# heliaxdev/kzg-setup-powersoftau

Hardware: AMD Instinct MI355X
Metric: G1+G2 points decompressed+checked/sec, 2^27 BLS12-381 PoT (higher is better)
Workload: dtype u32 (381-bit Montgomery, 14 x 28-bit limbs)

## Files before the change

### kzg-setup-powersoftau_amd/csrc/curve.hpp

```cpp
#pragma once
#include "fp381.hpp"

namespace kzgpot {

template <typename F>
struct jac {
  F x, y, z;
};

template <const auto& K>
KZG_DEV void f_subk(fp& r, const fp& a, const fp& b) { fp_subk_nr<K>(r, a, b); }
template <int S>
KZG_DEV void f_shl(fp& r, const fp& a) { fp_shl_nr<S>(r, a); }
KZG_DEV void f_mul_sub(fp& r, const fp& a, const fp& b, const fp& c, const fp& d) {
  fp nd;
  fp_negk_nr<BlsFp::KB_4_28>(nd, d);
  fp_mul_sum2(r, a, b, c, nd);
}

KZG_DEV void jac_dbl(jac<fp>& p) {
  fp a, b, d, e, t;
  fp_sqr(a, p.x);
  fp_sqr(b, p.y);
  fp_shl_nr<2>(t, p.x);
  fp_mul(d, t, b);
  fp_mul3_nr(e, a);
  fp_norm(e, e);
  fp_shl_nr<1>(t, p.y);
  fp_mul(p.z, t, p.z);
  fp_sqr(a, e);
  fp_shl_nr<1>(t, d);
  fp_subk_nr<BlsFp::KB_8_29>(p.x, a, t);
  fp_mul3_nr(t, d);
  fp_subk_nr<BlsFp::KB_8_30>(t, a, t);
  fp_mul_add8sqr(d, e, t, b);
  fp_negk_nr<BlsFp::KB_2_28>(p.y, d);
}

constexpr int F30_ZK = 16;
KZG_DEV void f_one(f30& r) { f30_set(r, ONE30); }

KZG_DEV void jac_dbl_w(jac<f30>& p) {
  f30 a, b, d, e, t;
  f30_sqr(a, p.x);
  f30_sqr(b, p.y);
  f30_mul(d, p.x, b);
  f30_mul3(e, a);
  f30_norm(e, e);
  f30_mul(p.z, p.y, p.z);
  f30_sqr<-2>(p.x, e, d);
  f30_sub(t, p.x, d);
  f30_norm<1>(t, t);
  f30_mul_addsqr(d, e, t, b);
  f30_neg(p.y, d);
}

KZG_DEV void jac_tpl_affine_w(jac<f30>& p) {
  f30 xx, yy, m, mm, s, e, ee, t, u, n;
  f30_sqr(xx, p.x);
  f30_sqr(yy, p.y);
  f30_sqr(t, yy);
  f30_mul3(m, xx);
  f30_norm(m, m);
  f30_sqr(mm, m);
  f30_mul(s, p.x, yy);
  f30_mul3(s, s);
  f30_norm(s, s);
  f30_sub(s, s, mm);
  f30_norm(e, s);
  f30_sqr(ee, e);
  f30_add(s, m, e);
  f30_norm(s, s);
  f30_sqr<-1, -1>(s, s, mm, ee);
  f30_sub(s, s, t);
  f30_norm(u, s);
  f30_neg(n, u);
  f30_mul_sum2(s, p.x, ee, yy, n);
  f30_norm<2>(p.x, s);
  f30_sub(t, t, u);
  f30_norm(t, t);
  f30_neg(n, ee);
  f30_mul_sum2(s, u, t, e, n);
  f30_mul(s, p.y, s);
  f30_norm<3>(p.y, s);
  f30_norm<1>(p.z, e);
}

template <typename Load>
KZG_DEV void jac_madd_w(jac<f30>& p, Load&& load) {
  f30 z1z1, h, r, t;
  {
    f30 x2, w2;
    load(x2, w2);
    f30_sqr(z1z1, p.z);
    f30_mul<-1>(h, x2, z1z1, p.x);
    f30_mul(t, w2, p.z);
    f30_mul<-1>(r, t, z1z1, p.y);
  }
  const bool z1zero = f30_is_zero<F30_ZK>(p.z);
  const bool same = !z1zero && f30_is_zero<F30_ZK>(h) && f30_is_zero<F30_ZK>(r);
  if (__builtin_expect(z1zero || same, 0)) {
    if (same) {
      jac_dbl_w(p);
    } else {
      load(p.x, p.y);
      f_one(p.z);
    }
    return;
  }
  f30 hh, j;
  f30_sqr(hh, h);
  f30_dbl(t, p.z);
  f30_mul(p.z, t, h);
  f30_norm<2>(hh, hh);
  f30_mul(j, h, hh);
  f30_mul(hh, p.x, hh);
  f30_sqr<-1, -2>(t, r, j, hh);
  f30_sub(hh, hh, t);
  f30_norm(hh, hh);
  f30_norm<1>(r, r);
  f30_norm<1>(h, p.y);
  f30_neg(j, j);
  f30_mul_sum2(p.y, r, hh, h, j);
  p.x = t;
}

template <const auto& K>
KZG_DEV void f2_mul_lz(fp2& r, const fp2& a, const fp2& b) {
  fp nb1, c0;
  fp_negk_nr<K>(nb1, b.c1);
  fp_mul_sum2(c0, a.c0, b.c0, a.c1, nb1);
  fp_mul_sum2(r.c1, a.c0, b.c1, a.c1, b.c0);
  r.c0 = c0;
}
template <const auto& K>
KZG_DEV void f2_sqr_lz(fp2& r, const fp2& a) {
  fp s, d, t;
  fp_add_nr(s, a.c0, a.c1);
  fp_subk_nr<K>(d, a.c0, a.c1);
  fp_shl_nr<1>(t, a.c0);
  fp_mul(r.c1, t, a.c1);
  fp_mul(r.c0, s, d);
}
template <const auto& K>
KZG_DEV void f2_subk(fp2& r, const fp2& a, const fp2& b) {
  fp_subk_nr<K>(r.c0, a.c0, b.c0);
  fp_subk_nr<K>(r.c1, a.c1, b.c1);
}
template <int S>
KZG_DEV void f2_shl(fp2& r, const fp2& a) {
  fp_shl_nr<S>(r.c0, a.c0);
  fp_shl_nr<S>(r.c1, a.c1);
}
KZG_DEV void f2_add_nr(fp2& r, const fp2& a, const fp2& b) {
  fp_add_nr(r.c0, a.c0, b.c0);
  fp_add_nr(r.c1, a.c1, b.c1);
}
KZG_DEV void f2_norm(fp2& r, const fp2& a) {
  fp_norm(r.c0, a.c0);
  fp_norm(r.c1, a.c1);
}

template <bool W = false>
KZG_DEV void jac_dbl(jac<fp2>& p) {
  fp2 b, a, d, t;
  if constexpr (W) {
    f2_sqr_lz<BlsFp::KB_32_29>(b, p.y);
    f2_mul_lz<BlsFp::KB_16_28>(p.z, p.y, p.z);
  } else {
    f2_sqr_lz<BlsFp::KB_32_28>(b, p.y);
    f2_shl<1>(t, p.y);
    f2_mul_lz<BlsFp::KB_16_28>(p.z, t, p.z);
  }
  f2_sqr_lz<BlsFp::KB_16_28>(a, p.x);
  if constexpr (W) {
    f2_mul_lz<BlsFp::KB_2_28>(d, p.x, b);
  } else {
    f2_shl<2>(t, p.x);
    f2_mul_lz<BlsFp::KB_2_28>(d, t, b);
  }
  fp_mul3_nr(a.c0, a.c0);
  fp_mul3_nr(a.c1, a.c1);
  f2_norm(a, a);
  f2_sqr_lz<BlsFp::KB_4_28>(t, a);
  f2_shl<1>(p.x, d);
  f2_subk<BlsFp::KB_4_29>(p.x, t, p.x);
  f2_norm(p.x, p.x);
  f2_subk<BlsFp::KB_8_28>(d, d, p.x);
  if constexpr (W) f2_shl<1>(a, a);
  fp u, s, n, c0;
  fp_negk_nr<BlsFp::KB_16_30>(u, d.c1);
  fp_add_nr(s, b.c0, b.c1);
  if constexpr (W) {
    fp_subk_nr<BlsFp::KB_2_28>(n, b.c1, b.c0);
    fp_norm(n, n);
  } else {
    fp_subk_nr<BlsFp::KB_2_28>(n, b.c0, b.c1);
    fp_norm(n, n);
    fp_shl_nr<3>(n, n);
    fp_negk_nr<BlsFp::KB_64_31>(n, n);
    fp_norm(n, n);
  }
  fp_mul_sum3(c0, a.c0, d.c0, a.c1, u, s, n);
  if constexpr (W) {
    fp_negk_nr<BlsFp::KB_2_28>(n, b.c1);
  } else {
    fp_shl_nr<3>(n, b.c1);
    fp_negk_nr<BlsFp::KB_16_31>(n, n);
    fp_norm(n, n);
  }
  fp_shl_nr<1>(s, b.c0);
  fp_mul_sum3(p.y.c1, a.c0, d.c1, a.c1, d.c0, s, n);
  p.y.c0 = c0;
}

template <bool W = false, typename Load>
KZG_DEV void jac_madd(jac<fp2>& p, Load&& load) {
  fp2 z1z1, h, r, t;
  {
    fp2 x2, y2;
    load(x2, y2);
    f2_sqr_lz<BlsFp::KB_16_28>(z1z1, p.z);
    f2_mul_lz<BlsFp::KB_2_28>(h, x2, z1z1);
    f2_subk<BlsFp::KB_32_28>(h, h, p.x);
    f2_norm(h, h);
    f2_mul_lz<BlsFp::KB_16_28>(t, y2, p.z);
    f2_mul_lz<BlsFp::KB_2_28>(t, t, z1z1);
    if constexpr (W)
      f2_subk<BlsFp::KB_32_29>(r, t, p.y);
    else
      f2_subk<BlsFp::KB_32_28>(r, t, p.y);
    f2_norm(r, r);
  }
  const bool z1zero = f_is_zero(p.z);
  const bool same = !z1zero && f_is_zero(h) && f_is_zero(r);
  if (__builtin_expect(z1zero || same, 0)) {
    if (same) {
      jac_dbl<W>(p);
    } else {
      load(p.x, p.y);
      f_one(p.z);
    }
    return;
  }
  fp2 hh, j;
  f2_sqr_lz<BlsFp::KB_64_28>(hh, h);
  f2_shl<1>(t, p.z);
  f2_mul_lz<BlsFp::KB_64_28>(p.z, t, h);
  f2_shl<2>(hh, hh);
  f2_mul_lz<BlsFp::KB_8_30>(j, h, hh);
  f2_mul_lz<BlsFp::KB_8_30>(hh, p.x, hh);
  f2_sqr_lz<BlsFp::KB_64_28>(t, r);
  if constexpr (!W) f2_shl<2>(t, t);
  f2_subk<BlsFp::KB_2_28>(t, t, j);
  f2_shl<1>(h, hh);
  f2_subk<BlsFp::KB_4_29>(t, t, h);
  f2_norm(t, t);
  f2_subk<BlsFp::KB_32_28>(hh, hh, t);
  f2_shl<1>(r, r);
  f2_mul_lz<BlsFp::KB_64_30>(hh, r, hh);
  f2_shl<1>(h, p.y);
  f2_mul_lz<BlsFp::KB_2_28>(j, h, j);
  f2_subk<BlsFp::KB_4_28>(p.y, hh, j);
  f2_norm(p.y, p.y);
  p.x = t;
}

template <typename Load>
KZG_DEV void jac_tpl_affine_w(jac<fp2>& p, Load&& load) {
  fp2 yy, m, s, ee, t;
  load(p.x, p.y);
  f2_sqr_lz<BlsFp::KB_2_28>(m, p.x);
  f2_sqr_lz<BlsFp::KB_4_29>(yy, p.y);
  f2_mul_lz<BlsFp::KB_2_28>(p.z, p.x, yy);
  fp_mul3_nr(m.c0, m.c0);
  fp_mul3_nr(m.c1, m.c1);
  f2_norm(m, m);
  f2_sqr_lz<BlsFp::KB_4_28>(t, m);
  fp_mul3_nr(p.z.c0, p.z.c0);
  fp_mul3_nr(p.z.c1, p.z.c1);
  f2_subk<BlsFp::KB_2_28>(p.z, p.z, t);
  f2_norm(p.z, p.z);
  f2_add_nr(s, m, p.z);
  f2_norm(s, s);
  f2_sqr_lz<BlsFp::KB_32_28>(s, s);
  f2_subk<BlsFp::KB_2_28>(s, s, t);
  f2_sqr_lz<BlsFp::KB_16_28>(ee, p.z);
  f2_subk<BlsFp::KB_4_28>(s, s, ee);
  f2_sqr_lz<BlsFp::KB_2_28>(t, yy);
  f2_subk<BlsFp::KB_2_28>(s, s, t);
  f2_norm(s, s);
  f2_subk<BlsFp::KB_64_28>(t, t, s);
  f2_norm(t, t);
  f2_mul_lz<BlsFp::KB_128_28>(t, s, t);
  f2_mul_lz<BlsFp::KB_64_28>(yy, yy, s);
  f2_mul_lz<BlsFp::KB_2_28>(m, p.z, ee);
  f2_subk<BlsFp::KB_2_28>(t, t, m);
  f2_norm(t, t);
  load(p.x, p.y);
  f2_mul_lz<BlsFp::KB_2_28>(p.x, p.x, ee);
  f2_subk<BlsFp::KB_2_28>(p.x, p.x, yy);
  f2_norm(p.x, p.x);
  f2_mul_lz<BlsFp::KB_8_28>(p.y, p.y, t);
}

template <typename F, typename Load>
KZG_DEV void jac_madd(jac<F>& p, Load&& load) {
  F z1z1, h, r, t;
  {
    F x2, y2;
    load(x2, y2);
    f_sqr(z1z1, p.z);
    f_mul(h, x2, z1z1);
    f_subk<BlsFp::KB_128_31>(h, h, p.x);
    f_norm(h, h);
    f_mul(t, y2, p.z);
    f_mul(t, t, z1z1);
    f_subk<BlsFp::KB_64_31>(r, t, p.y);
    f_norm(r, r);
  }
  const bool z1zero = f_is_zero(p.z);
  const bool same = !z1zero && f_is_zero(h) && f_is_zero(r);
  if (__builtin_expect(z1zero || same, 0)) {
    if (same) {
      jac_dbl(p);
    } else {
      load(p.x, p.y);
      f_one(p.z);
    }
    return;
  }
  F hh, j;
  f_sqr(hh, h);
  f_shl<1>(t, p.z);
  f_mul(p.z, t, h);
  f_shl<2>(hh, hh);
  f_norm(hh, hh);
  f_mul(j, h, hh);
  f_mul(hh, p.x, hh);
  f_sqr(t, r);
  f_shl<2>(t, t);
  f_subk<BlsFp::KB_32_28>(t, t, j);
  f_shl<1>(h, hh);
  f_subk<BlsFp::KB_64_29>(t, t, h);
  f_norm(t, t);
  f_subk<BlsFp::KB_128_28>(hh, hh, t);
  f_norm(hh, hh);
  f_shl<1>(r, r);
  f_shl<1>(h, p.y);
  f_mul_sub(p.y, r, hh, h, j);
  p.x = t;
}

template <typename F, typename Load>
KZG_DEV void mul_abs_u_affine(jac<F>& acc, Load&& load) {
  static_assert(((BLS_ABS_U >> (BLS_ABS_U_BITS - 2)) & 3) == 3, "|u| starts with the bits 11");
  if constexpr (__is_same(F, f30)) {
    load(acc.x, acc.y);
    jac_tpl_affine_w(acc);
#pragma unroll 1
    for (int b = BLS_ABS_U_BITS - 3; b >= 0; b--) {
      jac_dbl_w(acc);
      if ((BLS_ABS_U >> b) & 1) jac_madd_w(acc, load);
    }
  } else {
    static_assert(__is_same(F, fp2), "the fast ladders run on f30 (G1) and fp2 (G2)");
    auto loadw = [&](fp2& x, fp2& w) {
      load(x, w);
      f2_shl<1>(w, w);
    };
    jac_tpl_affine_w(acc, loadw);
#pragma unroll 1
    for (int b = BLS_ABS_U_BITS - 3; b >= 0; b--) {
      jac_dbl<true>(acc);
      if ((BLS_ABS_U >> b) & 1) jac_madd<true>(acc, loadw);
    }
  }
}
template <typename F>
KZG_DEV bool jac_eq_affine(const jac<F>& p, const F& x, const F& y) {
  F z2, t;
  f_sqr(z2, p.z);
  f_mul(t, x, z2);
  f_subk<BlsFp::KB_128_31>(t, t, p.x);
  bool ok = f_is_zero(t);
  f_mul(z2, z2, p.z);
  f_mul(t, y, z2);
  f_subk<BlsFp::KB_128_31>(t, t, p.y);
  ok = ok && f_is_zero(t);
  return ok && !f_is_zero(p.z);
}

KZG_DEV bool jac_eq_affine(const jac<fp2>& p, const fp2& x, const fp2& y) {
  fp2 z2, t;
  f2_sqr_lz<BlsFp::KB_16_28>(z2, p.z);
  f2_mul_lz<BlsFp::KB_2_28>(t, x, z2);
  f2_subk<BlsFp::KB_32_28>(t, t, p.x);
  bool ok = f_is_zero(t);
  f2_mul_lz<BlsFp::KB_16_28>(z2, z2, p.z);
  f2_mul_lz<BlsFp::KB_2_28>(t, y, z2);
  f2_subk<BlsFp::KB_32_29>(t, t, p.y);
  ok = ok && f_is_zero(t);
  return ok && !f_is_zero(p.z);
}

template <typename F, typename Load>
KZG_DEV bool in_subgroup_ref(Load&& load) {
  jac<F> acc;
  load(acc.x, acc.y);
  f_one(acc.z);
#pragma unroll 1
  for (int b = FR_R_BITS - 2; b >= 0; b--) {
    jac_dbl(acc);
    const uint32_t word = FR_R[b >> 5];
    if ((word >> (b & 31)) & 1) jac_madd(acc, load);
  }
  return f_is_zero(acc.z);
}

KZG_DEV bool jac_eq_affine(const jac<f30>& p, const f30& x, const f30& w) {
  f30 z2, t;
  f30_sqr(z2, p.z);
  f30_mul(t, x, z2);
  f30_sub(t, t, p.x);
  bool ok = f30_is_zero<F30_ZK>(t);
  f30_mul(z2, z2, p.z);
  f30_mul(t, w, z2);
  f30_sub(t, t, p.y);
  ok = ok && f30_is_zero<F30_ZK>(t);
  return ok && !f30_is_zero<F30_ZK>(p.z);
}

template <typename LoadRow, typename Park, typename LoadQZ>
KZG_DEV bool in_subgroup_fast_g1(LoadRow&& load_row, Park&& park, LoadQZ&& load_qz) {
  jac<f30> q;
  int src = 0;
  auto load = [&](f30& bx, f30& bw) { load_row(src, bx, bw); };
#pragma unroll 1
  for (int pass = 0; pass < 2; pass++) {
    src = __builtin_amdgcn_readfirstlane(pass);
    mul_abs_u_affine(q, load);
    if (pass == 0) park(q);
  }
  {
    f30 z;
    load_qz(z);
    f30_mul(q.z, q.z, z);
  }
  f30 x, w, beta;
  load_row(0, x, w);
  f30_set(beta, BETA30);
  f30_mul(x, x, beta);
  f30_neg(w, w);
  return jac_eq_affine(q, x, w);
}

KZG_DEV void g2_psi(fp2& x, fp2& y) {
  fp cx1, t;
  fp_set(cx1, FP_PSI_CX1);
  fp_mul(t, x.c1, cx1);
  fp_mul(x.c1, x.c0, cx1);
  x.c0 = t;
  fp2 cy;
  fp_set(cy.c0, FP_PSI_CY0);
  fp_set(cy.c1, FP_PSI_CY1);
  fp zero;
  fp_zero(zero);
  fp_sub_red(y.c1, zero, y.c1);
  f_mul(y, y, cy);
}

template <typename Load>
KZG_DEV bool in_subgroup_fast_g2(Load&& load) {
  jac<fp2> q;
  mul_abs_u_affine(q, load);
  fp2 x, y;
  load(x, y);
  g2_psi(x, y);
  fp2_neg_red(y, y);
  f2_shl<1>(y, y);
  return jac_eq_affine(q, x, y);
}

KZG_DEV void f_inv(fp& r, const fp& a) {
  fp t;
  fp_pow_pm3d4(t, a);
  fp_sqr(t, t);
  fp_sqr(t, t);
  fp_mul(r, t, a);
}
KZG_DEV void f_inv(fp2& r, const fp2& a) {
  fp n, t;
  fp_sqr(n, a.c0);
  fp_sqr(t, a.c1);
  fp_add(n, n, t);
  f_inv(n, n);
  fp_mul(r.c0, a.c0, n);
  fp_mul(t, a.c1, n);
  fp_zero(n);
  fp_sub_red(r.c1, n, t);
}

template <typename F>
KZG_DEV void to_affine(F& x, F& y, const jac<F>& p) {
  F zi, z2;
  f_inv(zi, p.z);
  f_sqr(z2, zi);
  f_mul(x, p.x, z2);
  f_mul(z2, z2, zi);
  f_mul(y, p.y, z2);
}

}
```

### kzg-setup-powersoftau_amd/csrc/fp381.hpp

```cpp
#pragma once
#include <hip/hip_runtime.h>
#include <stdint.h>

#include <utility>

#include "bls12_381_consts.hpp"
#include "bn254_consts.hpp"

#define KZG_DEV __device__ __forceinline__

#ifndef KZG_FPOP
#define KZG_FPOP(kind) ((void)0)
#endif

namespace kzgpot {

enum class FpOp { Mul, Sqr, MulSum2, MulSum3, MulAddSqr, Mul30, Sqr30, Mul30Sum2, Mul30AddSqr, Count };

constexpr uint32_t LMASK = (1u << 28) - 1;

template <class Tr>
struct Fe {
  uint32_t v[Tr::NL];
};
// ... 195 lines not shown
KZG_DEV void fp_mul3_nr(Fe<Tr>& r, const Fe<Tr>& a) {
#pragma unroll
  for (int i = 0; i < Tr::NL; i++) r.v[i] = (a.v[i] << 1) + a.v[i];
}
template <uint32_t C>
KZG_DEV uint32_t lit_sub(uint32_t b) {
  uint32_t r;
  asm("v_sub_u32_e32 %0, %1, %2" : "=v"(r) : "n"(C), "v"(b));
  return r;
}
template <uint32_t C>
KZG_DEV uint32_t lit_add(uint32_t a) {
  uint32_t r;
  asm("v_add_u32_e32 %0, %1, %2" : "=v"(r) : "n"(C), "v"(a));
  return r;
}
template <const auto& K, class Tr, size_t... I>
KZG_DEV void subk_lit(Fe<Tr>& r, const Fe<Tr>& a, const Fe<Tr>& b, std::index_sequence<I...>) {
  ((r.v[I] = lit_add<K[I]>(a.v[I]) - b.v[I]), ...);
}
template <const auto& K, class Tr, size_t... I>
KZG_DEV void negk_lit(Fe<Tr>& r, const Fe<Tr>& b, std::index_sequence<I...>) {
  ((r.v[I] = lit_sub<K[I]>(b.v[I])), ...);
}
template <const auto& K, class Tr>
KZG_DEV void fp_subk_nr(Fe<Tr>& r, const Fe<Tr>& a, const Fe<Tr>& b) {
  subk_lit<K>(r, a, b, std::make_index_sequence<Tr::NL>{});
}
template <const auto& K, class Tr>
KZG_DEV void fp_negk_nr(Fe<Tr>& r, const Fe<Tr>& b) {
  negk_lit<K>(r, b, std::make_index_sequence<Tr::NL>{});
}
template <class Tr>
KZG_DEV void fp_norm(Fe<Tr>& r, const Fe<Tr>& a) {
  uint32_t c = 0;
#pragma unroll
  for (int i = 0; i < Tr::NL - 1; i++) {
    const uint32_t t = a.v[i] + c;
    r.v[i] = t & Tr::MASK;
    c = t >> Tr::LB;
  }
  r.v[Tr::NL - 1] = a.v[Tr::NL - 1] + c;
}
template <class Tr>
KZG_DEV void fp_select(Fe<Tr>& r, bool c, const Fe<Tr>& a, const Fe<Tr>& b) {
#pragma unroll
  for (int i = 0; i < Tr::NL; i++) r.v[i] = c ? a.v[i] : b.v[i];
}

template <class Tr>
KZG_DEV void fp_half(Fe<Tr>& r, const Fe<Tr>& a) {
  const uint32_t odd = 0u - (a.v[0] & 1u);
  Fe<Tr> t;
  uint32_t c = 0;
#pragma unroll
  for (int i = 0; i < Tr::NL - 1; i++) {
    const uint32_t s = a.v[i] + (Tr::P[i] & odd) + c;
    t.v[i] = s & Tr::MASK;
    c = s >> Tr::LB;
  }
  t.v[Tr::NL - 1] = a.v[Tr::NL - 1] + (Tr::P[Tr::NL - 1] & odd) + c;
#pragma unroll
  for (int i = 0; i < Tr::NL - 1; i++) r.v[i] = (t.v[i] >> 1) | ((t.v[i + 1] & 1u) << (Tr::LB - 1));
  r.v[Tr::NL - 1] = t.v[Tr::NL - 1] >> 1;
}

template <class Tr>
KZG_DEV bool fp_sub_const_borrow(Fe<Tr>& d, const Fe<Tr>& a, const uint32_t (&k)[Tr::NL]) {
  int32_t br = 0;
#pragma unroll
  for (int i = 0; i < Tr::NL; i++) {
    const int32_t t = (int32_t)a.v[i] - (int32_t)k[i] + br;
    d.v[i] = (uint32_t)t & Tr::MASK;
    br = t >> Tr::LB;
  }
  return br != 0;
}
template <class Tr>
KZG_DEV void fp_reduce_once(Fe<Tr>& r, const Fe<Tr>& a) {
  Fe<Tr> d;
  const bool b = fp_sub_const_borrow(d, a, Tr::P);
  fp_select(r, b, a, d);
}
template <class Tr>
KZG_DEV void fp_reduce_canon(Fe<Tr>& r, const Fe<Tr>& a) {
  Fe<Tr> x = a, d;
#define KZG_RED_STEP(K)                          \
  {                                              \
    const bool b = fp_sub_const_borrow(d, x, K); \
    fp_select(x, b, x, d);                       \
  }
  KZG_RED_STEP(Tr::P_X128)
  KZG_RED_STEP(Tr::P_X64)
  KZG_RED_STEP(Tr::P_X32)
  KZG_RED_STEP(Tr::P_X16)
  KZG_RED_STEP(Tr::P_X8)
  KZG_RED_STEP(Tr::P_X4)
  KZG_RED_STEP(Tr::P_X2)
  KZG_RED_STEP(Tr::P_X1)
#undef KZG_RED_STEP
  r = x;
}
template <class Tr>
KZG_DEV void fp_canon(Fe<Tr>& r, const Fe<Tr>& a) {
  Fe<Tr> n;
  fp_norm(n, a);
  fp_reduce_canon(r, n);
}
template <class Tr>
KZG_DEV bool fp_is_zero_canon(const Fe<Tr>& c) {
  uint32_t o = 0;
#pragma unroll
  for (int i = 0; i < Tr::NL; i++) o |= c.v[i];
  return o == 0;
}
template <class Tr>
KZG_DEV bool fp_is_zero(const Fe<Tr>& a) {
  constexpr int N = Tr::NL;
  const uint32_t kc = ((a.v[0] & Tr::MASK) * (0u - Tr::PINV)) & Tr::MASK;
  const bool maybe = kc < 256u;
  if (__builtin_amdgcn_ballot_w64(maybe) == 0) return false;
  if (!maybe) return false;
  Fe<Tr> n;
  fp_norm(n, a);
  const uint32_t k = (uint32_t)((double)(n.v[N - 1] + 1u) * Tr::INV_RHO);
  uint64_t c = 0;
  uint32_t diff = 0;
#pragma unroll
  for (int i = 0; i < N - 1; i++) {
    c += (uint64_t)k * Tr::P[i];
    diff |= ((uint32_t)c & Tr::MASK) ^ n.v[i];
    c >>= Tr::LB;
  }
  c += (uint64_t)k * Tr::P[N - 1];
  diff |= (uint32_t)c ^ n.v[N - 1];
  return diff == 0;
}
template <class Tr>
KZG_DEV bool fp_eq(const Fe<Tr>& a, const Fe<Tr>& b) {
  Fe<Tr> d;
  fp_subk_nr<Tr::KB_EQ>(d, a, b);
  return fp_is_zero(d);
}
template <class Tr>
KZG_DEV bool fp_lt_canon(const Fe<Tr>& a, const Fe<Tr>& b) {
  Fe<Tr> d;
  return fp_sub_const_borrow(d, a, b.v);
}
template <class Tr>
KZG_DEV void fp_neg_canon(Fe<Tr>& r, const Fe<Tr>& c) {
  int32_t br = 0;
  const bool z = fp_is_zero_canon(c);
#pragma unroll
  for (int i = 0; i < Tr::NL; i++) {
    const int32_t t = (int32_t)Tr::P[i] - (int32_t)c.v[i] + br;
    r.v[i] = z ? 0u : ((uint32_t)t & Tr::MASK);
    br = t >> Tr::LB;
  }
}

template <class Tr>
KZG_DEV void fp_add(Fe<Tr>& r, const Fe<Tr>& a, const Fe<Tr>& b) {
  Fe<Tr> t;
  fp_add_nr(t, a, b);
  fp_norm(r, t);
}

template <class Tr>
KZG_DEV void fp_from_words(Fe<Tr>& r, const uint32_t (&w)[Tr::NW]) {
#pragma unroll
  for (int k = 0; k < Tr::NL; k++) {
    const int bit = Tr::LB * k, i = bit >> 5, off = bit & 31;
    const uint32_t lo = i < Tr::NW ? w[i] >> off : 0u;
    const uint32_t hi = (off > 32 - Tr::LB && i + 1 < Tr::NW) ? (w[i + 1] << (32 - off)) : 0u;
    r.v[k] = (lo | hi) & Tr::MASK;
  }
}
template <class Tr>
KZG_DEV void fp_to_words(uint32_t (&w)[Tr::NW], const Fe<Tr>& c) {
#pragma unroll
  for (int j = 0; j < Tr::NW; j++) {
    const int bit = 32 * j, k = bit / Tr::LB, off = bit % Tr::LB;
    uint32_t v = c.v[k] >> off;
    if (k + 1 < Tr::NL) v |= c.v[k + 1] << (Tr::LB - off);
    if (2 * Tr::LB - off < 32 && k + 2 < Tr::NL) v |= c.v[k + 2] << (2 * Tr::LB - off);
    w[j] = v;
  }
}
template <class Tr>
KZG_DEV bool words_geq_p_t(const uint32_t (&v)[Tr::NW]) {
  uint32_t br = 0;
#pragma unroll
  for (int i = 0; i < Tr::NW; i++) (void)__builtin_subc(v[i], Tr::P_WORDS[i], br, &br);
  return br == 0;
}
KZG_DEV bool words_geq_p(const uint32_t (&v)[BlsFp::NW]) { return words_geq_p_t<BlsFp>(v); }

template <class Tr>
KZG_DEV void fp_to_mont(Fe<Tr>& r, const Fe<Tr>& canon) {
  Fe<Tr> r2;
  fp_set(r2, Tr::R2);
  fp_mul(r, canon, r2);
}
template <class Tr>
KZG_DEV void fp_from_mont(Fe<Tr>& canon, const Fe<Tr>& a) {
  Fe<Tr> one;
  fp_zero(one);
  one.v[0] = 1;
  fp_mul(canon, a, one);
  fp_reduce_once(canon, canon);
}

constexpr int N30 = 13;
struct f30 {
  int32_t v[N30];
};
KZG_DEV int32_t sext30(uint32_t x) { return __builtin_amdgcn_sbfe((int32_t)x, 0, 30); }

#define KZG_F30_VV(k) "v_mad_i64_i32 %[c], %[o], %[x" #k "], %[y" #k "], %[c]\n\t"
#define KZG_F30_VK(k) "v_mad_i64_i32 %[c], %[o], %[m" #k "], %[p" #k "], %[c]\n\t"
#define KZG_F30_VV_IN(k) [x##k] "v"(x[k]), [y##k] "v"(y[k])
#define KZG_F30_VK_IN(k) [m##k] "v"(m[k]), [p##k] "s"(p[k])
#define KZG_F30_S1(M) M(0)
#define KZG_F30_S2(M) KZG_F30_S1(M) M(1)
#define KZG_F30_S3(M) KZG_F30_S2(M) M(2)
#define KZG_F30_S4(M) KZG_F30_S3(M) M(3)
#define KZG_F30_S5(M) KZG_F30_S4(M) M(4)
#define KZG_F30_S6(M) KZG_F30_S5(M) M(5)
#define KZG_F30_S7(M) KZG_F30_S6(M) M(6)
#define KZG_F30_S8(M) KZG_F30_S7(M) M(7)
#define KZG_F30_S9(M) KZG_F30_S8(M) M(8)
#define KZG_F30_S10(M) KZG_F30_S9(M) M(9)
#define KZG_F30_S11(M) KZG_F30_S10(M) M(10)
#define KZG_F30_S12(M) KZG_F30_S11(M) M(11)
#define KZG_F30_S13(M) KZG_F30_S12(M) M(12)
#define KZG_F30_L1(M) M(0)
#define KZG_F30_L2(M) KZG_F30_L1(M), M(1)
#define KZG_F30_L3(M) KZG_F30_L2(M), M(2)
#define KZG_F30_L4(M) KZG_F30_L3(M), M(3)
#define KZG_F30_L5(M) KZG_F30_L4(M), M(4)
#define KZG_F30_L6(M) KZG_F30_L5(M), M(5)
#define KZG_F30_L7(M) KZG_F30_L6(M), M(6)
#define KZG_F30_L8(M) KZG_F30_L7(M), M(7)
#define KZG_F30_L9(M) KZG_F30_L8(M), M(8)
#define KZG_F30_L10(M) KZG_F30_L9(M), M(9)
#define KZG_F30_L11(M) KZG_F30_L10(M), M(10)
#define KZG_F30_L12(M) KZG_F30_L11(M), M(11)
#define KZG_F30_L13(M) KZG_F30_L12(M), M(12)
#define KZG_F30_TS0
#define KZG_F30_TS1 "v_mad_i64_i32 %[c], %[o], %[t0], %[k0], %[c]\n\t"
#define KZG_F30_TS2 KZG_F30_TS1 "v_mad_i64_i32 %[c], %[o], %[t1], %[k1], %[c]\n\t"
#define KZG_F30_TIN0
#define KZG_F30_TIN1 , [t0] "v"(t[0]), [k0] "n"(K0)
#define KZG_F30_TIN2 KZG_F30_TIN1, [t1] "v"(t[1]), [k1] "n"(K1)
#define KZG_F30_RUN(n, T, W) \
  if constexpr (Cnt == n)    \
    asm(KZG_F30_S##n(KZG_F30_##T) KZG_F30_TS##W : [c] "+v"(c), [o] "=&s"(carry_out) : KZG_F30_L##n(KZG_F30_##T##_IN) KZG_F30_TIN##W);
#define KZG_F30_RUNS12(T, W) \
  KZG_F30_RUN(1, T, W) KZG_F30_RUN(2, T, W) KZG_F30_RUN(3, T, W) KZG_F30_RUN(4, T, W) KZG_F30_RUN(5, T, W) \
  KZG_F30_RUN(6, T, W) KZG_F30_RUN(7, T, W) KZG_F30_RUN(8, T, W) KZG_F30_RUN(9, T, W) KZG_F30_RUN(10, T, W) \
  KZG_F30_RUN(11, T, W) KZG_F30_RUN(12, T, W)
#define KZG_F30_RUNS13(T, W) KZG_F30_RUNS12(T, W) KZG_F30_RUN(13, T, W)
template <int Cnt, bool Zero = false>
KZG_DEV int64_t mad_i64_run(const int32_t (&x)[13], const int32_t (&y)[13], int64_t c) {
  static_assert(Cnt >= 0 && Cnt <= 13, "a statement takes 30 operands");
  static_assert(!Zero || Cnt == 1 || Cnt == 2, "a column 0");
  [[maybe_unused]] uint64_t carry_out;
  if constexpr (Zero && Cnt == 1) {
    asm("v_mad_i64_i32 %[c], %[o], %[x0], %[y0], 0" : [c] "=v"(c), [o] "=s"(carry_out) : KZG_F30_VV_IN(0));
  } else if constexpr (Zero) {
    asm("v_mad_i64_i32 %[c], %[o], %[x0], %[y0], 0\n\t" KZG_F30_VV(1)
        : [c] "=&v"(c), [o] "=&s"(carry_out)
        : KZG_F30_L2(KZG_F30_VV_IN));
  } else {
    KZG_F30_RUNS13(VV, 0)
  }
  return c;
}
template <int Cnt, int K0 = 0, int K1 = 0>
KZG_DEV int64_t mad_i64_run_k(const int32_t (&m)[13], const int32_t (&p)[13], int64_t c, const int32_t (&t)[2] = {0, 0}) {
  static_assert(Cnt >= 0 && Cnt + (K0 != 0) + (K1 != 0) <= 14 && (K0 != 0 || K1 == 0), "a statement takes 30 operands");
  static_assert(K0 >= -16 && K0 <= 64 && K1 >= -16 && K1 <= 64, "a tail's factor is an inline constant");
  [[maybe_unused]] uint64_t carry_out;
  if constexpr (K1 != 0) {
    static_assert(Cnt >= 1, "an upper column");
    KZG_F30_RUNS12(VK, 2)
  } else if constexpr (K0 != 0) {
    static_assert(Cnt >= 1, "an upper column");
    KZG_F30_RUNS13(VK, 1)
  } else {
    KZG_F30_RUNS13(VK, 0)
  }
  return c;
}
#undef KZG_F30_RUNS13
#undef KZG_F30_RUNS12
#undef KZG_F30_RUN
#undef KZG_F30_TIN2
#undef KZG_F30_TIN1
#undef KZG_F30_TIN0
#undef KZG_F30_TS2
#undef KZG_F30_TS1
#undef KZG_F30_TS0
constexpr int F30_NV = 20;

template <int I, int End, class F>
KZG_DEV void f30_static_for(F&& f) {
  if constexpr (I < End) {
    f(std::integral_constant<int, I>{});
    f30_static_for<I + 1, End>(f);
  }
}
template <int Off, int Cnt, bool Zero = false>
KZG_DEV int64_t f30_run(const int32_t (&x)[F30_NV], const int32_t (&y)[F30_NV], int64_t acc) {
  int32_t xs[N30], ys[N30];
#pragma unroll
  for (int j = 0; j < Cnt; j++) xs[j] = x[Off + j], ys[j] = y[Off + j];
  return mad_i64_run<Cnt, Zero>(xs, ys, acc);
}
template <int NV, int NK, bool Zero = false, int K0 = 0, int K1 = 0>
KZG_DEV int64_t f30_col(const int32_t (&x)[F30_NV], const int32_t (&y)[F30_NV], const int32_t (&m)[N30],
                        const int32_t (&p)[N30], int64_t acc, const int32_t (&t)[2] = {0, 0}) {
  static_assert(NV >= 0 && NV <= F30_NV && NK >= 0 && NK <= N30, "column");
  if constexpr (Zero) {
    static_assert(NK == 0, "column 0");
    return f30_run<0, NV, true>(x, y, acc);
  }
  constexpr int V0 = NV > 13 ? (NV + 1) / 2 : NV;
  acc = f30_run<0, V0>(x, y, acc);
  acc = f30_run<V0, NV - V0>(x, y, acc);
  return mad_i64_run_k<NK, K0, K1>(m, p, acc, t);
}
template <int I>
KZG_DEV int64_t f30_col_end(int64_t acc, int32_t (&m)[N30], f30& r) {
  if constexpr (I < N30) {
    m[I] = sext30((uint32_t)acc * PINV30);
    acc += (int64_t)m[I] * P30[0];
  } else {
    r.v[I - N30] = sext30((uint32_t)acc);
    acc += (int64_t)1 << 29;
  }
  return acc >> 30;
}
template <int I, int NV, int K0 = 0, int K1 = 0>
KZG_DEV int64_t f30_column(const int32_t (&x)[F30_NV], const int32_t (&y)[F30_NV], int64_t acc, int32_t (&m)[N30],
                           f30& r, const int32_t (&t0)[N30] = {}, const int32_t (&t1)[N30] = {}) {
  constexpr int j0 = I < N30 ? 0 : I - (N30 - 1), nk = (I < N30 ? I - 1 : N30 - 1) - j0 + 1;
  int32_t mm[N30], pp[N30];
#pragma unroll
  for (int k = 0; k < nk; k++) mm[k] = m[j0 + k], pp[k] = P30[I - j0 - k];
  if constexpr (I < N30 || K0 == 0) {
    acc = f30_col<NV, nk, I == 0>(x, y, mm, pp, acc);
  } else {
    const int32_t t[2] = {t0[I - N30], t1[I - N30]};
    acc = f30_col<NV, nk, false, K0, K1>(x, y, mm, pp, acc, t);
  }
  return f30_col_end<I>(acc, m, r);
}
template <int K0, int K1>
KZG_DEV int32_t f30_top(int64_t acc, const f30& t0, const f30& t1) {
  if constexpr (K0 == 0) return (int32_t)acc;
  else if constexpr (K1 == 0) return (int32_t)acc + K0 * t0.v[N30 - 1];
  else return (int32_t)acc + K0 * t0.v[N30 - 1] + K1 * t1.v[N30 - 1];
}
template <int K0 = 0, int K1 = 0>
KZG_DEV void f30_mul(f30& r, const f30& a, const f30& b, const f30& t0 = f30{}, const f30& t1 = f30{}) {
  KZG_FPOP(FpOp::Mul30);
  constexpr int N = N30;
  int32_t m[N];
  int64_t acc = 0;
  f30_static_for<0, 2 * N - 1>([&](auto col) __attribute__((always_inline)) {
    constexpr int i = decltype(col)::value;
    constexpr int j0 = i < N ? 0 : i - (N - 1), n = (i < N ? i - 1 : N - 1) - j0 + 1;
    int32_t x[F30_NV], y[F30_NV];
#pragma unroll
    for (int j = 0; j < n; j++) x[j] = a.v[j0 + j], y[j] = b.v[i - j0 - j];
    if constexpr (i < N) x[n] = a.v[i], y[n] = b.v[0];
    acc = f30_column<i, n + (i < N), K0, K1>(x, y, acc, m, r, t0.v, t1.v);
  });
  r.v[N - 1] = f30_top<K0, K1>(acc, t0, t1);
}
template <int K0 = 0, int K1 = 0>
KZG_DEV void f30_sqr(f30& r, const f30& a, const f30& t0 = f30{}, const f30& t1 = f30{}) {
  KZG_FPOP(FpOp::Sqr30);
  constexpr int N = N30;
  int32_t d[N], m[N];
#pragma unroll
  for (int j = 0; j < N; j++) d[j] = dbl_i32(a.v[j]);
  int64_t acc = 0;
  f30_static_for<0, 2 * N - 1>([&](auto col) __attribute__((always_inline)) {
    constexpr int i = decltype(col)::value;
    constexpr int j0 = i < N ? 0 : i - (N - 1);
    constexpr int nc = (i + 1) / 2 - j0, sq = (i & 1) == 0;
    int32_t x[F30_NV], y[F30_NV];
#pragma unroll
    for (int j = 0; j < nc; j++) x[j] = a.v[j0 + j], y[j] = d[i - j0 - j];
    if constexpr (sq) x[nc] = y[nc] = a.v[i / 2];
    acc = f30_column<i, nc + sq, K0, K1>(x, y, acc, m, r, t0.v, t1.v);
  });
  r.v[N - 1] = f30_top<K0, K1>(acc, t0, t1);
}
KZG_DEV void f30_mul_sum2(f30& r, const f30& a, const f30& b, const f30& c, const f30& d) {
  KZG_FPOP(FpOp::Mul30Sum2);
  constexpr int N = N30;
  int32_t m[N];
  int64_t acc = 0;
#pragma unroll
  for (int i = 0; i < 2 * N - 1; i++) {
    const int j0 = i < N ? 0 : i - (N - 1);
    const int j1 = i < N ? i - 1 : N - 1;
#pragma unroll
    for (int j = j0; j <= j1; j++) {
      acc += (int64_t)a.v[j] * b.v[i - j];
      acc += (int64_t)c.v[j] * d.v[i - j];
      acc += (int64_t)m[j] * P30[i - j];
    }
    if (i < N) {
      acc += (int64_t)a.v[i] * b.v[0];
      acc += (int64_t)c.v[i] * d.v[0];
      m[i] = sext30((uint32_t)acc * PINV30);
      acc += (int64_t)m[i] * P30[0];
    } else {
      r.v[i - N] = sext30((uint32_t)acc);
      acc += (int64_t)1 << 29;
    }
    acc >>= 30;
  }
  r.v[N - 1] = (int32_t)acc;
}
KZG_DEV void f30_mul_addsqr(f30& r, const f30& a, const f30& b, const f30& c) {
  KZG_FPOP(FpOp::Mul30AddSqr);
  constexpr int N = N30;
  int32_t c2[N], m[N];
#pragma unroll
  for (int j = 0; j < N; j++) c2[j] = dbl_i32(c.v[j]);
  int64_t acc = 0;
  f30_static_for<0, 2 * N - 1>([&](auto col) __attribute__((always_inline)) {
    constexpr int i = decltype(col)::value;
    constexpr int j0 = i < N ? 0 : i - (N - 1), n = (i < N ? i - 1 : N - 1) - j0 + 1;
    constexpr int nc = (i + 1) / 2 - j0, sq = (i & 1) == 0;
    int32_t x[F30_NV], y[F30_NV];
#pragma unroll
    for (int j = 0; j < n; j++) x[j] = a.v[j0 + j], y[j] = b.v[i - j0 - j];
#pragma unroll
    for (int j = 0; j < nc; j++) x[n + j] = c.v[j0 + j], y[n + j] = c2[i - j0 - j];
    if constexpr (sq) x[n + nc] = y[n + nc] = c.v[i / 2];
    if constexpr (i < N) x[n + nc + sq] = a.v[i], y[n + nc + sq] = b.v[0];
    acc = f30_column<i, n + nc + sq + (i < N)>(x, y, acc, m, r);
  });
  r.v[N - 1] = (int32_t)acc;
}
KZG_DEV void f30_set(f30& r, const int32_t (&c)[N30]) {
#pragma unroll
  for (int i = 0; i < N30; i++) r.v[i] = c[i];
}
KZG_DEV void f30_add(f30& r, const f30& a, const f30& b) {
#pragma unroll
  for (int i = 0; i < N30; i++) r.v[i] = a.v[i] + b.v[i];
}
KZG_DEV void f30_sub(f30& r, const f30& a, const f30& b) {
#pragma unroll
  for (int i = 0; i < N30; i++) r.v[i] = a.v[i] - b.v[i];
}
KZG_DEV void f30_neg(f30& r, const f30& a) {
#pragma unroll
  for (int i = 0; i < N30; i++) r.v[i] = -a.v[i];
}
KZG_DEV void f30_dbl(f30& r, const f30& a) {
#pragma unroll
  for (int i = 0; i < N30; i++) r.v[i] = dbl_i32(a.v[i]);
}
KZG_DEV void f30_mul3(f30& r, const f30& a) {
#pragma unroll
  for (int i = 0; i < N30; i++) r.v[i] = dbl_i32(a.v[i]) + a.v[i];
}
template <int S = 0>
KZG_DEV void f30_norm(f30& r, const f30& a) {
  static_assert(S >= 0 && S <= 3, "shift");
  int32_t c = 0;
#pragma unroll
  for (int k = 0; k < N30 - 1; k++) {
    const int32_t lo = __builtin_amdgcn_sbfe(a.v[k], 0, 30 - S);
    const int32_t cn = (a.v[k] + (1 << (29 - S))) >> (30 - S);
    r.v[k] = S == 1 ? dbl_i32(lo) + c : S ? (int32_t)((uint32_t)lo << S) + c : lo + c;
    c = cn;
  }
  r.v[N30 - 1] = (S == 1 ? dbl_i32(a.v[N30 - 1]) : (int32_t)((uint32_t)a.v[N30 - 1] << S)) + c;
}
template <int K>
KZG_DEV bool f30_is_zero(const f30& a) {
  const int32_t k = sext30((uint32_t)a.v[0] * (0u - PINV30));
  const bool maybe = (uint32_t)(k + K) <= 2u * K;
  if (__builtin_amdgcn_ballot_w64(maybe) == 0) return false;
  if (!maybe) return false;
  int64_t c = 0;
  uint32_t diff = 0;
#pragma unroll
  for (int i = 0; i < N30; i++) {
    c += (int64_t)a.v[i] - (int64_t)k * P30[i];
    if (i < N30 - 1) {
      diff |= (uint32_t)c & ((1u << 30) - 1);
      c >>= 30;
    }
  }
  return diff == 0 && c == 0;
}

KZG_DEV void f30_from_fp(f30& r, const fp& a) {
  fp n;
  fp_norm(n, a);
  int32_t c = 0;
#pragma unroll
  for (int k = 0; k < N30; k++) {
    const int bit = 30 * k, i = bit / 28, off = bit % 28;
    uint32_t u = (n.v[i] >> off) | (i + 1 < NL ? n.v[i + 1] << (28 - off) : 0u);
    if (k < N30 - 1) {
      const int32_t t = (int32_t)(u & ((1u << 30) - 1)) + c;
      c = (t + (1 << 29)) >> 30;
      r.v[k] = sext30((uint32_t)t);
    } else {
      r.v[k] = (int32_t)u + c;
    }
  }
}
KZG_DEV void fp_from_f30(fp& r, const f30& z) {
  uint32_t u[N30];
  int32_t c = 0;
#pragma unroll
  for (int k = 0; k < N30; k++) {
    const int32_t t = z.v[k] + P30[k] + c;
    if (k < N30 - 1) {
      u[k] = (uint32_t)t & ((1u << 30) - 1);
      c = t >> 30;
    } else {
      u[k] = (uint32_t)t;
    }
  }
#pragma unroll
  for (int j = 0; j < NL; j++) {
    const int bit = 28 * j, i = bit / 30, off = bit % 30;
    uint32_t v = u[i] >> off;
    if (off > 2 && i + 1 < N30) v |= u[i + 1] << (30 - off);
    r.v[j] = j < NL - 1 ? v & LMASK : v;
  }
  fp_reduce_once(r, r);
}

template <int H>
KZG_DEV void f30_from_mont(f30& r, const fp& a) {
  static_assert(H == 1 || H == 2, "halvings");
  fp t;
  fp_half(t, a);
  if (H == 2) fp_half(t, t);
  f30_from_fp(r, t);
}
template <int H>
KZG_DEV void fp_mont_from_f30(fp& r, const f30& z) {
  static_assert(H == 1 || H == 2, "doublings");
  fp_from_f30(r, z);
#pragma unroll
  for (int k = 0; k < H; k++) {
    fp_add(r, r, r);
    fp_reduce_once(r, r);
  }
}

template <class Tr>
struct SqrtSchedule {
  int32_t step[Tr::SQRT_STEPS + 1];
  constexpr SqrtSchedule() : step{} {
    for (int s = 0; s < Tr::SQRT_STEPS; s++) step[s] = (Tr::SQRT_STEP_SQ[s] & 0xff) | (Tr::SQRT_STEP_IDX[s] * 256);
    step[Tr::SQRT_STEPS] = 0;
  }
};
template <class Tr>
__constant__ constexpr SqrtSchedule<Tr> kSqrtSchedule{};
KZG_DEV int sched_nsq(int32_t packed) { return __builtin_amdgcn_readfirstlane(packed & 0xff); }
KZG_DEV int sched_idx(int32_t packed) { return __builtin_amdgcn_readfirstlane(packed >> 8); }

constexpr bool bls_sqrt_table_is(const int16_t (&e)[8]) {
  constexpr int16_t want[8] = {1, 3, 7, 9, 11, 13, 21, 255};
  for (int k = 0; k < 8; k++)
    if (e[k] != want[k]) return false;
  return true;
}
KZG_DEV void fp_pow_pm3d4_30(fp& r, const fp& a_in) {
  typedef uint32_t v8u __attribute__((ext_vector_type(8)));
  static_assert(BlsFp::SQRT_TABLE == 8, "table held as one 8-wide register vector per limb");
  static_assert(bls_sqrt_table_is(BlsFp::SQRT_TABLE_EXP), "the chain below builds exactly this table");
  v8u tab[N30];
  auto put = [&](int e, const f30& x) {
#pragma unroll
    for (int k = 0; k < N30; k++) tab[k][e] = (uint32_t)x.v[k];
  };
  f30 a, a2, a4, t, u;
  f30_from_fp(a, a_in);
  put(0, a);
  f30_sqr(a2, a);
  f30_mul(t, a, a2);
  put(1, t);
  f30_sqr(a4, a2);
  f30_mul(t, t, a4);
  put(2, t);
  f30_mul(t, t, a2);
  put(3, t);
  f30_mul(t, t, a2);
  put(4, t);
  f30_mul(t, t, a2);
  put(5, t);
  f30_sqr(a4, a4);
  f30_mul(u, t, a4);
  put(6, u);
  f30_mul(t, t, a2);
  u = t;
#pragma unroll 1
  for (int k = 0; k < 4; k++) f30_sqr(u, u);
  f30_mul(u, u, t);
  put(7, u);
  f30 acc;
#pragma unroll
  for (int k = 0; k < N30; k++) acc.v[k] = (int32_t)tab[k][BlsFp::SQRT_STEP_IDX[0]];
  int32_t step = kSqrtSchedule<BlsFp>.step[1];
#pragma unroll 1
  for (int s = 1; s < BlsFp::SQRT_STEPS; s++) {
    const int nsq = sched_nsq(step), idx = sched_idx(step);
    step = kSqrtSchedule<BlsFp>.step[s + 1];
#pragma unroll 1
    for (int k = 0; k < nsq; k++) f30_sqr(acc, acc);
    if (idx >= 0) {
#pragma unroll
      for (int k = 0; k < N30; k++) t.v[k] = (int32_t)tab[k][idx];
      f30_mul(acc, acc, t);
    }
  }
#pragma unroll
  for (int k = 0; k < N30; k++) t.v[k] = POW30_OUT[k];
  f30_mul(acc, acc, t);
  fp_from_f30(r, acc);
}

template <class Tr>
KZG_DEV void fp_pow_pm3d4_window(Fe<Tr>& r, const Fe<Tr>& a) {
  static_assert(Tr::SQRT_TABLE == 8, "table held as one 8-wide register vector per limb");
  static_assert(Tr::SQRT_TABLE_EXP[0] == 1 && Tr::SQRT_TABLE_EXP[7] == 15, "sliding-window table a, a^3, .., a^15");
  typedef uint32_t v8u __attribute__((ext_vector_type(8)));
  v8u tab[Tr::NL];
  Fe<Tr> a2, t = a;
  fp_sqr(a2, a);
#pragma unroll
  for (int k = 0; k < Tr::NL; k++) tab[k][0] = a.v[k];
#pragma clang loop unroll(full)
  for (int e = 1; e < Tr::SQRT_TABLE; e++) {
    fp_mul(t, t, a2);
#pragma unroll
    for (int k = 0; k < Tr::NL; k++) tab[k][e] = t.v[k];
  }
  Fe<Tr> acc;
#pragma unroll
  for (int k = 0; k < Tr::NL; k++) acc.v[k] = tab[k][Tr::SQRT_STEP_IDX[0]];
  int32_t step = kSqrtSchedule<Tr>.step[1];
#pragma unroll 1
  for (int s = 1; s < Tr::SQRT_STEPS; s++) {
    const int nsq = sched_nsq(step), idx = sched_idx(step);
    step = kSqrtSchedule<Tr>.step[s + 1];
#pragma unroll 1
    for (int k = 0; k < nsq; k++) fp_sqr(acc, acc);
    if (idx >= 0) {
#pragma unroll
      for (int k = 0; k < Tr::NL; k++) t.v[k] = tab[k][idx];
      fp_mul(acc, acc, t);
    }
  }
  r = acc;
}
template <class Tr>
KZG_DEV void fp_pow_pm3d4(Fe<Tr>& r, const Fe<Tr>& a) {
  if constexpr (__is_same(Tr, BlsFp)) fp_pow_pm3d4_30(r, a);
  else fp_pow_pm3d4_window(r, a);
}

KZG_DEV void fp_cond_sub_2p(fp& r, const fp& a) {
  fp d;
  const bool b = fp_sub_const_borrow(d, a, BlsFp::P_X2);
  fp_select(r, b, a, d);
}
KZG_DEV void fp_add_red(fp& r, const fp& a, const fp& b) {
  fp t;
  fp_add_nr(t, a, b);
  fp_norm(t, t);
  fp_cond_sub_2p(r, t);
}
KZG_DEV void fp_sub_red(fp& r, const fp& a, const fp& b) {
  fp d, e;
  int32_t br = 0;
#pragma unroll
  for (int i = 0; i < NL; i++) {
    const int32_t t = (int32_t)a.v[i] - (int32_t)b.v[i] + br;
    d.v[i] = (uint32_t)t & LMASK;
    br = t >> 28;
  }
  uint32_t c = 0;
#pragma unroll
  for (int i = 0; i < NL; i++) {
    const uint32_t t = d.v[i] + BlsFp::P_X2[i] + c;
    e.v[i] = t & LMASK;
    c = t >> 28;
  }
  fp_select(r, br != 0, e, d);
}

struct fp2 {
  fp c0, c1;
};
KZG_DEV void f_mul(fp& r, const fp& a, const fp& b) { fp_mul(r, a, b); }
KZG_DEV void f_sqr(fp& r, const fp& a) { fp_sqr(r, a); }
KZG_DEV bool f_is_zero(const fp& a) { return fp_is_zero(a); }
KZG_DEV void f_one(fp& r) { fp_set(r, BlsFp::ONE); }
KZG_DEV void f_norm(fp& r, const fp& a) { fp_norm(r, a); }

KZG_DEV void f_mul(fp2& r, const fp2& a, const fp2& b) {
  fp nb1, c0;
  fp_negk_nr<BlsFp::KB_4_28>(nb1, b.c1);
  fp_mul_sum2(c0, a.c0, b.c0, a.c1, nb1);
  fp_mul_sum2(r.c1, a.c0, b.c1, a.c1, b.c0);
  r.c0 = c0;
}
KZG_DEV void f_sqr(fp2& r, const fp2& a) {
  fp s, d, t;
  fp_add_nr(s, a.c0, a.c1);
  fp_subk_nr<BlsFp::KB_4_28>(d, a.c0, a.c1);
// ... 18 lines not shown
```

Measured before the change: 68.81 million.

## Fold point negations into the G1 ladder and check only x in subgroup test

The G1 |u| ladder no longer negates y after each doubling. It tracks the sign by parity and negates the loaded affine y in madd when needed, which removes one f30_neg per doubling. The final endomorphism check compares only x coordinates, which drops two muls and a compare, and rejects x=0 explicitly. f30_mul_sum2 is rewritten to use the column-based f30_column path with a larger F30_NV. This risks correctness if the sign-parity bookkeeping or the x-only comparison is subtly wrong (x-only equality accepts ±point).

```diff
diff --git a/kzg-setup-powersoftau_amd/csrc/curve.hpp b/kzg-setup-powersoftau_amd/csrc/curve.hpp
--- a/kzg-setup-powersoftau_amd/csrc/curve.hpp
+++ b/kzg-setup-powersoftau_amd/csrc/curve.hpp
@@ -40,6 +40,7 @@
 constexpr int F30_ZK = 16;
 KZG_DEV void f_one(f30& r) { f30_set(r, ONE30); }
 
+template <bool Neg = true>
 KZG_DEV void jac_dbl_w(jac<f30>& p) {
   f30 a, b, d, e, t;
   f30_sqr(a, p.x);
@@ -52,7 +53,8 @@
   f30_sub(t, p.x, d);
   f30_norm<1>(t, t);
   f30_mul_addsqr(d, e, t, b);
-  f30_neg(p.y, d);
+  if constexpr (Neg) f30_neg(p.y, d);
+  else p.y = d;
 }
 
 KZG_DEV void jac_tpl_affine_w(jac<f30>& p) {
@@ -87,11 +89,12 @@
 }
 
 template <typename Load>
-KZG_DEV void jac_madd_w(jac<f30>& p, Load&& load) {
+KZG_DEV void jac_madd_w(jac<f30>& p, Load&& load, bool neg = false) {
   f30 z1z1, h, r, t;
   {
     f30 x2, w2;
     load(x2, w2);
+    if (neg) f30_neg(w2, w2);
     f30_sqr(z1z1, p.z);
     f30_mul<-1>(h, x2, z1z1, p.x);
     f30_mul(t, w2, p.z);
@@ -104,6 +107,7 @@
       jac_dbl_w(p);
     } else {
       load(p.x, p.y);
+      if (neg) f30_neg(p.y, p.y);
       f_one(p.z);
     }
     return;
@@ -356,12 +360,13 @@
 KZG_DEV void mul_abs_u_affine(jac<F>& acc, Load&& load) {
   static_assert(((BLS_ABS_U >> (BLS_ABS_U_BITS - 2)) & 3) == 3, "|u| starts with the bits 11");
   if constexpr (__is_same(F, f30)) {
+    static_assert(BLS_ABS_U_BITS % 2 == 0, "an even number of doublings: bit b's is number BLS_ABS_U_BITS - 2 - b");
     load(acc.x, acc.y);
     jac_tpl_affine_w(acc);
 #pragma unroll 1
     for (int b = BLS_ABS_U_BITS - 3; b >= 0; b--) {
-      jac_dbl_w(acc);
-      if ((BLS_ABS_U >> b) & 1) jac_madd_w(acc, load);
+      jac_dbl_w<false>(acc);
+      if ((BLS_ABS_U >> b) & 1) jac_madd_w(acc, load, (b & 1) != 0);
     }
   } else {
     static_assert(__is_same(F, fp2), "the fast ladders run on f30 (G1) and fp2 (G2)");
@@ -418,17 +423,11 @@
   return f_is_zero(acc.z);
 }
 
-KZG_DEV bool jac_eq_affine(const jac<f30>& p, const f30& x, const f30& w) {
+KZG_DEV bool jac_eq_affine_x(const jac<f30>& p, const f30& x) {
   f30 z2, t;
   f30_sqr(z2, p.z);
-  f30_mul(t, x, z2);
-  f30_sub(t, t, p.x);
-  bool ok = f30_is_zero<F30_ZK>(t);
-  f30_mul(z2, z2, p.z);
-  f30_mul(t, w, z2);
-  f30_sub(t, t, p.y);
-  ok = ok && f30_is_zero<F30_ZK>(t);
-  return ok && !f30_is_zero<F30_ZK>(p.z);
+  f30_mul<-1>(t, x, z2, p.x);
+  return f30_is_zero<F30_ZK>(t) && !f30_is_zero<F30_ZK>(p.z);
 }
 
 template <typename LoadRow, typename Park, typename LoadQZ>
@@ -449,10 +448,10 @@
   }
   f30 x, w, beta;
   load_row(0, x, w);
+  const bool x_zero = f30_is_zero<F30_ZK>(x);
   f30_set(beta, BETA30);
   f30_mul(x, x, beta);
-  f30_neg(w, w);
-  return jac_eq_affine(q, x, w);
+  return jac_eq_affine_x(q, x) && !x_zero;
 }
 
 KZG_DEV void g2_psi(fp2& x, fp2& y) {
diff --git a/kzg-setup-powersoftau_amd/csrc/f30_codec_hooks.hip b/kzg-setup-powersoftau_amd/csrc/f30_codec_hooks.hip
--- /dev/null
+++ b/kzg-setup-powersoftau_amd/csrc/f30_codec_hooks.hip
@@ -0,0 +1,83 @@
+#ifdef KZGPOT_TEST_HOOKS
+#include "../../tests/kzgpot_test_f30_codec_hooks.h"
+#include "curve.hpp"
+#include "device_rt.hpp"
+
+using namespace kzgpot;
+
+namespace {
+
+constexpr int kBlock = 256;
+constexpr int kIn = KZGPOT_F30_CODEC_IN * N30, kOut = KZGPOT_F30_CODEC_OUT * N30;
+
+__device__ __forceinline__ void f30_load(f30& x, const int32_t* p) {
+#pragma unroll
+  for (int k = 0; k < N30; k++) x.v[k] = p[k];
+}
+__device__ __forceinline__ void f30_store(int32_t* p, const f30& x) {
+#pragma unroll
+  for (int k = 0; k < N30; k++) p[k] = x.v[k];
+}
+
+template <int OP>
+__global__ void __launch_bounds__(kBlock) k_f30_codec_op(long n, const int32_t* __restrict__ in, int32_t* __restrict__ out) {
+  const long i = (long)blockIdx.x * kBlock + threadIdx.x;
+  if (i >= n) return;
+  const int32_t* src = in + kIn * i;
+  jac<f30> p;
+  f30_load(p.x, src);
+  f30_load(p.y, src + N30);
+  f30_load(p.z, src + 2 * N30);
+  auto load = [&](f30& x2, f30& w2) {
+    f30_load(x2, src + 3 * N30);
+    f30_load(w2, src + 4 * N30);
+  };
+  if (OP == KZGPOT_F30_CODEC_DBL_KEEP) jac_dbl_w<false>(p);
+  if (OP == KZGPOT_F30_CODEC_MADD) jac_madd_w(p, load, false);
+  if (OP == KZGPOT_F30_CODEC_MADD_NEG) jac_madd_w(p, load, true);
+  if (OP == KZGPOT_F30_CODEC_LADDER) mul_abs_u_affine(p, load);
+  if (OP == KZGPOT_F30_CODEC_SUBGROUP) {
+    jac<f30> q1;
+    auto load_row = [&](int row, f30& x, f30& w) {
+      if (row) x = q1.x, w = q1.y;
+      else load(x, w);
+    };
+    const bool ok = in_subgroup_fast_g1(load_row, [&](const jac<f30>& q) { q1 = q; }, [&](f30& z) { z = q1.z; });
+#pragma unroll
+    for (int k = 0; k < N30; k++) p.x.v[k] = p.y.v[k] = p.z.v[k] = 0;
+    p.x.v[0] = ok;
+  }
+  f30_store(out + kOut * i, p.x);
+  f30_store(out + kOut * i + N30, p.y);
+  f30_store(out + kOut * i + 2 * N30, p.z);
+}
+
+template <int OP>
+int run_op(long n, const int32_t* in, int32_t* out) {
+  if (device_count() <= 0) return KZGPOT_E_DEVICE;
+  const size_t bin = (size_t)n * kIn * sizeof(int32_t), bout = (size_t)n * kOut * sizeof(int32_t);
+  DevBuf din, dout;
+  if (din.alloc(bin) || dout.alloc(bout)) return KZGPOT_E_DEVICE;
+  HIP_TRY(hipMemcpy(din.p, in, bin, hipMemcpyHostToDevice));
+  const unsigned blocks = (unsigned)((n + kBlock - 1) / kBlock);
+  hipLaunchKernelGGL(k_f30_codec_op<OP>, dim3(blocks), dim3(kBlock), 0, nullptr, n, (const int32_t*)din.p, (int32_t*)dout.p);
+  HIP_TRY(hipGetLastError());
+  HIP_TRY(hipStreamSynchronize(nullptr));
+  HIP_TRY(hipMemcpy(out, dout.p, bout, hipMemcpyDeviceToHost));
+  return 0;
+}
+
+}
+
+extern "C" int kzgpot_test_f30_codec_op(int op, long n, const int32_t* in, int32_t* out) {
+  if (n <= 0 || n > (1 << 20) || !in || !out) return KZGPOT_E_INVALID_ARG;
+  switch (op) {
+    case KZGPOT_F30_CODEC_DBL_KEEP: return run_op<KZGPOT_F30_CODEC_DBL_KEEP>(n, in, out);
+    case KZGPOT_F30_CODEC_MADD: return run_op<KZGPOT_F30_CODEC_MADD>(n, in, out);
+    case KZGPOT_F30_CODEC_MADD_NEG: return run_op<KZGPOT_F30_CODEC_MADD_NEG>(n, in, out);
+    case KZGPOT_F30_CODEC_LADDER: return run_op<KZGPOT_F30_CODEC_LADDER>(n, in, out);
+    case KZGPOT_F30_CODEC_SUBGROUP: return run_op<KZGPOT_F30_CODEC_SUBGROUP>(n, in, out);
+    default: return KZGPOT_E_INVALID_ARG;
+  }
+}
+#endif
diff --git a/kzg-setup-powersoftau_amd/csrc/fp381.hpp b/kzg-setup-powersoftau_amd/csrc/fp381.hpp
--- a/kzg-setup-powersoftau_amd/csrc/fp381.hpp
+++ b/kzg-setup-powersoftau_amd/csrc/fp381.hpp
@@ -521,7 +521,7 @@
 #undef KZG_F30_TS2
 #undef KZG_F30_TS1
 #undef KZG_F30_TS0
-constexpr int F30_NV = 20;
+constexpr int F30_NV = 26;
 
 template <int I, int End, class F>
 KZG_DEV void f30_static_for(F&& f) {
@@ -624,27 +624,21 @@
   constexpr int N = N30;
   int32_t m[N];
   int64_t acc = 0;
-#pragma unroll
-  for (int i = 0; i < 2 * N - 1; i++) {
-    const int j0 = i < N ? 0 : i - (N - 1);
-    const int j1 = i < N ? i - 1 : N - 1;
-#pragma unroll
-    for (int j = j0; j <= j1; j++) {
-      acc += (int64_t)a.v[j] * b.v[i - j];
-      acc += (int64_t)c.v[j] * d.v[i - j];
-      acc += (int64_t)m[j] * P30[i - j];
-    }
-    if (i < N) {
-      acc += (int64_t)a.v[i] * b.v[0];
-      acc += (int64_t)c.v[i] * d.v[0];
-      m[i] = sext30((uint32_t)acc * PINV30);
-      acc += (int64_t)m[i] * P30[0];
-    } else {
-      r.v[i - N] = sext30((uint32_t)acc);
-      acc += (int64_t)1 << 29;
-    }
-    acc >>= 30;
-  }
+  f30_static_for<0, 2 * N - 1>([&](auto col) __attribute__((always_inline)) {
+    constexpr int i = decltype(col)::value;
+    constexpr int j0 = i < N ? 0 : i - (N - 1), n = (i < N ? i - 1 : N - 1) - j0 + 1;
+    int32_t x[F30_NV], y[F30_NV];
+#pragma unroll
+    for (int j = 0; j < n; j++) {
+      x[j] = a.v[j0 + j], y[j] = b.v[i - j0 - j];
+      x[n + j] = c.v[j0 + j], y[n + j] = d.v[i - j0 - j];
+    }
+    if constexpr (i < N) {
+      x[2 * n] = a.v[i], y[2 * n] = b.v[0];
+      x[2 * n + 1] = c.v[i], y[2 * n + 1] = d.v[0];
+    }
+    acc = f30_column<i, 2 * n + 2 * (i < N)>(x, y, acc, m, r);
+  });
   r.v[N - 1] = (int32_t)acc;
 }
 KZG_DEV void f30_mul_addsqr(f30& r, const f30& a, const f30& b, const f30& c) {
```

New measurement: 69.12 million, median of 6. Within noise of the previous version (+0.4%).
